# sharonct/CTPA-CLIP

Hardware: AMD Instinct MI355X
Metric: CT-report pairs/sec (contrastive step) (higher is better)
Workload: dtype bf16

## Files before the change

ctpa-clip_amd/csrc/gemm.hip:

```cpp
#include <algorithm>
#include "common.h"
#include "../../include/ctclip_hip.h"

int ctclip_gemm256(const ctclip_gemm_args* a, int split, int batch, void* stream);

namespace {

constexpr int BM = 128, BN = 128, BKT = 64, NTH = 256;
constexpr int KROW = BKT * 2 + 16;
constexpr int TILE_BYTES = 128 * KROW;
constexpr int SMEM_BYTES = 4 * TILE_BYTES;
constexpr int CS_LD = 132;

struct P {
  int64_t M, N, K;
  const u16* A; int64_t lda;
  const u16* B; int64_t ldb;
  const u16* B2;
  void* C; int64_t ldc; int c_f32;
  u16* C2; int64_t ldc2;
  const float* bias;
  const void* R; int64_t ldr; int r_f32;
  float alpha; int act; int accumulate; int split_k;
  int64_t sA, sB, sC, sC2, sR;
  int64_t kper;
  int r_f16;
};

__device__ __forceinline__ int mn_swz(int k) { return (k & 3) | (((k >> 3) & 1) << 2); }

template <bool KC>
__device__ __forceinline__ void gload(u32x4 (&r)[4], const u16* __restrict__ base, int64_t ld,
                                      int64_t rows, int64_t kend, int64_t row0, int64_t k0) {
  const int t = threadIdx.x;
  if constexpr (KC) {
    const int kc = t & 7;
    const int64_t gk = k0 + kc * 8;
#pragma unroll
    for (int i = 0; i < 4; ++i) {
      const int64_t gr = row0 + (t >> 3) + 32 * i;
      if (gr < rows && gk < kend) r[i] = *(const u32x4*)(base + gr * ld + gk);
      else r[i] = make_uint4(0, 0, 0, 0);
    }
  } else {
    const int mc = t & 15;
    const int64_t gm = row0 + mc * 8;
#pragma unroll
    for (int i = 0; i < 4; ++i) {
      const int64_t gk = k0 + (t >> 4) + 16 * i;
      if (gk < kend && gm < rows) r[i] = *(const u32x4*)(base + gk * ld + gm);
      else r[i] = make_uint4(0, 0, 0, 0);
    }
  }
}

template <bool KC>
__device__ __forceinline__ void swrite(char* tile, const u32x4 (&r)[4]) {
  const int t = threadIdx.x;
  if constexpr (KC) {
    const int kc = t & 7;
#pragma unroll
    for (int i = 0; i < 4; ++i) *(u32x4*)(tile + ((t >> 3) + 32 * i) * KROW + kc * 16) = r[i];
  } else {
    const int mc = t & 15, c32 = mc >> 1, half = mc & 1;
#pragma unroll
    for (int i = 0; i < 4; ++i) {
      const int kk = (t >> 4) + 16 * i;
      *(u32x4*)(tile + kk * 256 + ((((c32 ^ mn_swz(kk)) << 1) | half) << 4)) = r[i];
    }
  }
}
// ... 2 lines not shown
__device__ __forceinline__ bf16x8 frag(const char* tile, int r0, int s, int lane) {
  if constexpr (KC) {
    const int row = r0 + (lane & 15);
    return *(const bf16x8*)(tile + row * KROW + ((s * 4 + (lane >> 4)) << 4));
  } else {
    const int g = lane >> 4, i = lane & 15, q = i >> 2, p = i & 3;
    const int m = r0 + 4 * p;
    const int k1 = s * 32 + 8 * g + q, k2 = k1 + 4;
    const int c32 = m >> 4, within = (m & 15) * 2;
    const int o1 = k1 * 256 + ((c32 ^ mn_swz(k1)) << 5) + within;
    const int o2 = k2 * 256 + ((c32 ^ mn_swz(k2)) << 5) + within;
    s16x4 lo = __builtin_amdgcn_ds_read_tr16_b64_v4i16(LDS_PTR(s16x4, tile + o1));
    s16x4 hi = __builtin_amdgcn_ds_read_tr16_b64_v4i16(LDS_PTR(s16x4, tile + o2));
    typedef short s16x8 __attribute__((ext_vector_type(8)));
    s16x8 v = {lo[0], lo[1], lo[2], lo[3], hi[0], hi[1], hi[2], hi[3]};
    return __builtin_bit_cast(bf16x8, v);
  }
}

__device__ __forceinline__ void xcd_remap(int& tx, int& ty) {
  const int gx = gridDim.x, nwg = gridDim.x * gridDim.y;
  const int orig = blockIdx.y * gx + blockIdx.x;
  int id = orig;
  if (nwg >= 16) {
    const int xcd = orig & 7, q = nwg >> 3, r = nwg & 7;
    id = (xcd < r ? xcd * (q + 1) : r * (q + 1) + (xcd - r) * q) + (orig >> 3);
  }
  ty = id / gx;
  tx = id - ty * gx;
}

template <bool AK, bool BK, bool H16 = false>
__global__ __launch_bounds__(NTH, 2) void gemm_kernel(P p) {
  extern __shared__ __attribute__((aligned(16))) char smem[];
  const int lane = threadIdx.x & 63, w = threadIdx.x >> 6, wr = w >> 1, wc = w & 1;
  int tx, ty;
  xcd_remap(tx, ty);
  const int split = blockIdx.z % p.split_k, bidx = blockIdx.z / p.split_k;
  const int64_t m0 = (int64_t)ty * BM, n0 = (int64_t)tx * BN;
  const int64_t kbeg = split * p.kper;
  const int64_t kend = min(p.K, kbeg + p.kper);
  const u16* A = p.A + bidx * p.sA;
  const u16* B = p.B + bidx * p.sB;
#define AS(i) (smem + (i) * TILE_BYTES)
#define BS(i) (smem + (2 + (i)) * TILE_BYTES)

  f32x4 acc[4][4];
#pragma unroll
  for (int i = 0; i < 4; ++i)
#pragma unroll
    for (int j = 0; j < 4; ++j) acc[i][j] = f32x4{0.f, 0.f, 0.f, 0.f};

  u32x4 ra[4], rb[4];
  const int nk1 = kend > kbeg ? (int)((kend - kbeg + BKT - 1) / BKT) : 0;
  const int nk = p.B2 ? 2 * nk1 : nk1;
  const u16* B2 = p.B2 ? p.B2 + bidx * p.sB : nullptr;
  if (nk > 0) {
    gload<AK>(ra, A, p.lda, p.M, kend, m0, kbeg);
    gload<BK>(rb, B, p.ldb, p.N, kend, n0, kbeg);
    swrite<AK>(AS(0), ra);
    swrite<BK>(BS(0), rb);
  }
  __syncthreads();
  for (int kt = 0; kt < nk; ++kt) {
    const int cur = kt & 1;
    if (kt + 1 < nk) {
      const int kn = kt + 1 < nk1 ? kt + 1 : kt + 1 - nk1;
      gload<AK>(ra, A, p.lda, p.M, kend, m0, kbeg + (int64_t)kn * BKT);
      gload<BK>(rb, kt + 1 < nk1 ? B : B2, p.ldb, p.N, kend, n0, kbeg + (int64_t)kn * BKT);
    }
#pragma unroll
    for (int s = 0; s < 2; ++s) {
      bf16x8 af[4], bfr[4];
#pragma unroll
      for (int i = 0; i < 4; ++i) af[i] = frag<AK>(AS(cur), wr * 64 + i * 16, s, lane);
#pragma unroll
      for (int j = 0; j < 4; ++j) bfr[j] = frag<BK>(BS(cur), wc * 64 + j * 16, s, lane);
#pragma unroll
      for (int i = 0; i < 4; ++i)
#pragma unroll
        for (int j = 0; j < 4; ++j)
          acc[i][j] = mfma16<H16>(af[i], bfr[j], acc[i][j]);
    }
    if (kt + 1 < nk) {
      swrite<AK>(AS(cur ^ 1), ra);
      swrite<BK>(BS(cur ^ 1), rb);
    }
    __syncthreads();
  }

  float* cs = (float*)smem;
#pragma unroll
  for (int i = 0; i < 4; ++i)
#pragma unroll
    for (int j = 0; j < 4; ++j)
#pragma unroll
      for (int r = 0; r < 4; ++r)
        cs[(wr * 64 + i * 16 + (lane >> 4) * 4 + r) * CS_LD + wc * 64 + j * 16 + (lane & 15)] = acc[i][j][r];
  __syncthreads();

  const int t = threadIdx.x;
  if (p.act == 3) {
    const int row = t >> 1, half = t & 1;
    const int ncol = (int)min((int64_t)BN, p.N - n0);
    float best = -INFINITY, second = -INFINITY;
    int bi = 0x7fffffff;
    for (int c = half * 64; c < half * 64 + 64; ++c) {
      const float v = cs[row * CS_LD + c];
      if (c < ncol) {
        if (v > best) { second = best; best = v; bi = c; }
        else if (v > second) second = v;
      }
    }
    const int64_t gm = m0 + row;
    if (gm < p.M && half * 64 < ncol) {
      float2* out = (float2*)p.C + bidx * p.sC;
      out[gm * p.ldc + tx * 2 + half] = make_float2(best, __int_as_float((int)(n0 + bi)));
      if (p.C2) ((float*)p.C2)[bidx * p.sC2 + gm * p.ldc2 + tx * 2 + half] = second;
    }
    return;
  }
  const bool slab = p.split_k > 1;
// ... 243 lines not shown
    for (int j = 0; j < 4; ++j) { v[j] += a[j]; v[4 + j] += b[j]; }
  }
  if (drop) {
#pragma unroll
    for (int j = 0; j < 8; ++j) v[j] *= hid_keep(seed, r * cols + c + j, thresh, dscale);
  }
  if (p.R) {
    if (p.r_f32) {
      const float* Rp = (const float*)p.R + r * p.ldr + c;
      const f32x4 a = *(const f32x4*)Rp, b = *(const f32x4*)(Rp + 4);
#pragma unroll
      for (int j = 0; j < 4; ++j) { v[j] += a[j]; v[4 + j] += b[j]; }
    } else {
      float rr[8];
      unpack8(*(const u32x4*)((const u16*)p.R + r * p.ldr + c), rr);
#pragma unroll
      for (int j = 0; j < 8; ++j) v[j] += rr[j];
    }
  }
  if (p.act == 1) {
    if (p.C2) *(u32x4*)(p.C2 + r * p.ldc2 + c) = pack8(v);
#pragma unroll
    for (int j = 0; j < 8; ++j) v[j] = gelu_erf(v[j]);
  }
  if (p.c_f32) {
    float* Cf = (float*)p.C + r * p.ldc + c;
    if (p.accumulate) {
      const f32x4 a = *(const f32x4*)Cf, b = *(const f32x4*)(Cf + 4);
#pragma unroll
      for (int j = 0; j < 4; ++j) { v[j] += a[j]; v[4 + j] += b[j]; }
    }
    *(f32x4*)Cf = f32x4{v[0], v[1], v[2], v[3]};
    *(f32x4*)(Cf + 4) = f32x4{v[4], v[5], v[6], v[7]};
  } else {
    u16* Cb = (u16*)p.C + r * p.ldc + c;
    if (p.accumulate) {
      float rr[8];
      unpack8(*(const u32x4*)Cb, rr);
#pragma unroll
      for (int j = 0; j < 8; ++j) v[j] += rr[j];
    }
    *(u32x4*)Cb = pack8(v);
  }
  if (p.C2 && p.act == 0) *(u32x4*)(p.C2 + r * p.ldc2 + c) = pack8(v);
}

static bool s_smem_set = false;

}

extern "C" int ctclip_gemm(const ctclip_gemm_args* a, void* stream) {
  if (!a) return CT_EINVAL;
  if (a->M <= 0 || a->N <= 0 || a->K <= 0) return a->M == 0 || a->N == 0 ? 0 : CT_ESHAPE;
  const int split = a->split_k > 0 ? a->split_k : 1;
  if (split > 1 && !a->c_f32) return CT_EINVAL;
  if (a->act == 2 && !a->C2) return CT_EINVAL;
  CT_REQUIRE(aligned16(a->A) && aligned16(a->B) && aligned16(a->C), CT_EALIGN);
  CT_REQUIRE(a->lda % 8 == 0 && a->ldb % 8 == 0, CT_EALIGN);
  CT_REQUIRE(a->a_kcontig ? (a->K % 8 == 0) : (a->M % 8 == 0), CT_EALIGN);
  CT_REQUIRE(a->b_kcontig ? (a->K % 8 == 0) : (a->N % 8 == 0), CT_EALIGN);
  if (a->act != 3) {
    CT_REQUIRE(a->N % 8 == 0 && a->ldc % 8 == 0, CT_EALIGN);
    if (a->C2) CT_REQUIRE(aligned16(a->C2) && a->ldc2 % 8 == 0, CT_EALIGN);
    if (a->R) CT_REQUIRE(aligned16(a->R) && a->ldr % 8 == 0, CT_EALIGN);
  }
  if (a->act == 2) CT_REQUIRE(a->N % 64 == 0 && a->ldc2 % 8 == 0, CT_ESHAPE);
  if (a->act == 4) CT_REQUIRE(a->N % 32 == 0 && a->R && !a->r_f32 && !a->c_f32 && a->split_k <= 1, CT_EINVAL);
  if (a->act == 6)
    CT_REQUIRE(a->R && !a->r_f32 && !a->bias && !a->accumulate && !a->C2 && split == 1 && (a->batch <= 1), CT_EINVAL);
  if (a->act == 5)
    CT_REQUIRE(a->C2 && a->bias && aligned16(a->bias) && !a->R && !a->c_f32 && !a->accumulate && split == 1 &&
                   (a->batch <= 1) && a->N % 64 == 0 && a->n2 > 0 && a->n2 % 64 == 0 && a->n2 <= a->N,
               CT_EINVAL);
  if (a->B2) CT_REQUIRE(aligned16(a->B2) && a->act != 3, CT_EINVAL);
  if (a->A_lo || a->B_lo) {
    CT_REQUIRE(a->A_lo && a->B_lo && a->ab_f16 && aligned16(a->A_lo) && aligned16(a->B_lo) && a->K % 64 == 0,
               CT_EINVAL);
    CT_REQUIRE(a->a_kcontig && a->b_kcontig && !a->B2 && split == 1 && !a->accumulate && a->batch <= 1, CT_EINVAL);
    CT_REQUIRE(a->K < (int64_t)64 * 10000, CT_ESHAPE);
    if (a->act == 2)
      CT_REQUIRE(!a->c_f32 && !a->R && !a->bias && a->C3 && aligned16(a->C3) && a->ldc3 % 8 == 0 &&
                     (!a->C4 || (aligned16(a->C4) && a->ldc4 % 8 == 0)),
                 CT_EINVAL);
    else
      CT_REQUIRE(a->act == 0 && a->c_f32 && (!a->R || a->r_f32), CT_EINVAL);
    return ctclip_gemm256(a, 1, 1, stream);
  }
  if (a->ab_f16)
    CT_REQUIRE(a->a_kcontig && a->b_kcontig && !a->B2 && split == 1 && (a->act == 0 || a->act == 2 || a->act == 3) &&
                   !a->accumulate && (a->batch <= 1),
               CT_EINVAL);
  if (!a->B2 && a->act != 6) {
    const int b = a->batch > 0 ? a->batch : 1;
    const int64_t tiles256 = ((a->M + 255) / 256) * ((a->N + 255) / 256) * split * b;
    if (a->K % 64 == 0 && a->M >= 256 && a->N >= 256 && tiles256 >= 160 && (split == 1 || (a->K / split) >= 512) &&
        (!a->bias || aligned16(a->bias)))
      return ctclip_gemm256(a, split, b, stream);
  }
  if (a->act == 5) {
    ctclip_gemm_args g = *a;
    g.act = 0;
    g.bias = nullptr;
    g.C2 = nullptr;
    const int rc = ctclip_gemm(&g, stream);
    if (rc) return rc;
    return ctclip_l2norm_scale_fwd(a->C, a->ldc, a->M, a->n2 / 32, 32, a->bias, a->C2, a->ldc2, stream);
  }
  if (!s_smem_set) {
    (void)hipFuncSetAttribute((const void*)gemm_kernel<true, true>, hipFuncAttributeMaxDynamicSharedMemorySize, SMEM_BYTES);
    (void)hipFuncSetAttribute((const void*)gemm_kernel<true, false>, hipFuncAttributeMaxDynamicSharedMemorySize, SMEM_BYTES);
    (void)hipFuncSetAttribute((const void*)gemm_kernel<false, true>, hipFuncAttributeMaxDynamicSharedMemorySize, SMEM_BYTES);
    (void)hipFuncSetAttribute((const void*)gemm_kernel<false, false>, hipFuncAttributeMaxDynamicSharedMemorySize, SMEM_BYTES);
    (void)hipFuncSetAttribute((const void*)gemm_kernel<true, true, true>, hipFuncAttributeMaxDynamicSharedMemorySize, SMEM_BYTES);
    s_smem_set = true;
  }
  P p;
  p.M = a->M; p.N = a->N; p.K = a->K;
  p.A = (const u16*)a->A; p.lda = a->lda;
  p.B = (const u16*)a->B; p.ldb = a->ldb;
  p.B2 = (const u16*)a->B2;
  p.C = a->C; p.ldc = a->ldc; p.c_f32 = a->c_f32;
  p.C2 = (u16*)a->C2; p.ldc2 = a->ldc2;
  p.bias = a->bias;
  p.R = a->R; p.ldr = a->ldr; p.r_f32 = a->r_f32;
  p.alpha = a->alpha; p.act = a->act; p.accumulate = a->accumulate; p.split_k = split;
  p.sA = a->sA; p.sB = a->sB; p.sC = a->sC; p.sC2 = a->sC2; p.sR = a->sR;
  int64_t kper = (a->K + split - 1) / split;
  kper = (kper + BKT - 1) / BKT * BKT;
  p.kper = kper;
  p.r_f16 = a->r_f16;
  const int batch = a->batch > 0 ? a->batch : 1;
  hipStream_t st = (hipStream_t)stream;
  if (a->ab_f16) return launch<true, true, true>(p, batch, st);
  if (a->a_kcontig && a->b_kcontig) return launch<true, true>(p, batch, st);
  if (a->a_kcontig && !a->b_kcontig) return launch<true, false>(p, batch, st);
  if (!a->a_kcontig && a->b_kcontig) return launch<false, true>(p, batch, st);
  return launch<false, false>(p, batch, st);
}

extern "C" int ctclip_reduce_slabs_ep(const float* slabs, int64_t nslab, int64_t rows, int64_t cols, int64_t ld,
                                      const ctclip_gemm_args* a, void* stream) {
  if (rows == 0 || cols == 0) return 0;
  CT_REQUIRE(a && (a->act == 0 || a->act == 1), CT_EINVAL);
  CT_REQUIRE(cols % 8 == 0 && ld % 4 == 0 && a->ldc % 8 == 0 && aligned16(slabs) && aligned16(a->C), CT_EALIGN);
  if (a->bias) CT_REQUIRE(aligned16(a->bias), CT_EALIGN);
  if (a->R) CT_REQUIRE(aligned16(a->R) && a->ldr % 8 == 0, CT_EALIGN);
  if (a->C2) CT_REQUIRE(aligned16(a->C2) && a->ldc2 % 8 == 0, CT_EALIGN);
  P p{};
  p.C = a->C; p.ldc = a->ldc; p.c_f32 = a->c_f32;
  p.C2 = (u16*)a->C2; p.ldc2 = a->ldc2;
  p.bias = a->bias;
  p.R = a->R; p.ldr = a->ldr; p.r_f32 = a->r_f32;
  p.act = a->act; p.accumulate = a->accumulate;
  const int64_t total = rows * (cols / 8);
  hipLaunchKernelGGL(reduce_slabs_ep_kernel, dim3(cdiv(total, 256)), dim3(256), 0, (hipStream_t)stream, slabs, nslab,
                     rows, cols, ld, p);
  CT_CHECK_LAUNCH();
  return 0;
}

extern "C" int ctclip_reduce_slabs_ep_drop(const float* slabs, int64_t nslab, int64_t rows, int64_t cols, int64_t ld,
                                           const ctclip_gemm_args* a, float dp, uint64_t seed, void* stream) {
  if (rows == 0 || cols == 0) return 0;
  CT_REQUIRE(a && a->act == 0 && !a->accumulate && a->ldc == cols && dp >= 0.f && dp < 1.f, CT_EINVAL);
  CT_REQUIRE(cols % 8 == 0 && ld % 4 == 0 && aligned16(slabs) && aligned16(a->C), CT_EALIGN);
  if (a->bias) CT_REQUIRE(aligned16(a->bias), CT_EALIGN);
  if (a->R) CT_REQUIRE(aligned16(a->R) && a->ldr % 8 == 0, CT_EALIGN);
  if (a->C2) CT_REQUIRE(aligned16(a->C2) && a->ldc2 % 8 == 0, CT_EALIGN);
  P p{};
  p.C = a->C; p.ldc = a->ldc; p.c_f32 = a->c_f32;
  p.C2 = (u16*)a->C2; p.ldc2 = a->ldc2;
  p.bias = a->bias;
  p.R = a->R; p.ldr = a->ldr; p.r_f32 = a->r_f32;
// ... 92 lines not shown
```

ctpa-clip_amd/ctclip_mi355x/_lib.py:

```python
from __future__ import annotations

import ctypes
import os

import torch

_HERE = os.path.dirname(os.path.abspath(__file__))
LIB_PATH = os.environ.get('CTCLIP_HIP_LIB') or os.path.join(_HERE, 'libctclip_hip.so')
_LIB = None

c_i64 = ctypes.c_int64
c_i32 = ctypes.c_int32
c_f32 = ctypes.c_float
c_vp = ctypes.c_void_p


class SlabJob(ctypes.Structure):
    _fields_ = [('slabs', c_vp), ('nslab', c_i64), ('cols', c_i64), ('out', c_vp), ('accumulate', c_i32),
                ('pad', c_i32)]


ABI_VERSION = 2


# ... 102 lines not shown

class ClipLossExArgs(ctypes.Structure):
    _fields_ = [
        ('t_raw', c_vp), ('i_raw', c_vp), ('t_extra', c_vp), ('i_extra', c_vp), ('log_temp', c_vp),
        ('Vt', c_i32), ('Vi', c_i32), ('Bg', c_i32), ('Dl', c_i32),
        ('decoupled', c_i32), ('w_main', c_f32), ('w_multiview', c_f32),
        ('loss', c_vp), ('pair_loss', c_vp),
        ('dt_raw', c_vp), ('di_raw', c_vp), ('dt_extra', c_vp), ('di_extra', c_vp),
        ('dlogtemp', c_vp),
        ('ws', c_vp), ('ws_floats', c_i64),
    ]


class ClipLossTiledArgs(ctypes.Structure):
    _fields_ = ClipLossExArgs._fields_[:-1] + [('ws_bytes', c_i64), ('grad_row0', c_i32), ('grad_rows', c_i32)]


class MlmMaskArgs(ctypes.Structure):
    _fields_ = [
        ('ids', c_vp), ('B', c_i32), ('L', c_i32),
        ('num_tokens', c_i64), ('mask_token_id', c_i64), ('pad_token_id', c_i64),
        ('ignore', c_i64 * 32), ('n_ignore', c_i32), ('m_max', c_i32),
        ('mask_prob', ctypes.c_double), ('replace_prob', ctypes.c_double), ('random_token_prob', ctypes.c_double),
        ('seed', ctypes.c_uint64),
        ('masked_ids', c_vp), ('labels', c_vp), ('sel', c_vp),
    ]


_SIGS = {
    'ctclip_version': [],
    'ctclip_device_arch': [ctypes.c_char_p, c_i32],
    'ctclip_debug_hold_cus': [c_i32, c_i64, c_i32, c_vp],
    'ctclip_gemm': [ctypes.POINTER(GemmArgs), c_vp],
    'ctclip_gemm_ln': [ctypes.POINTER(GemmArgs), ctypes.POINTER(LnEpilogueArgs), c_vp],
    'ctclip_gemm_qkv_lnfold': [ctypes.POINTER(GemmArgs), c_vp, c_vp, c_vp, c_i32, c_vp],
    'ctclip_gemm_qkv_lnfold2': [ctypes.POINTER(GemmArgs), c_vp, c_vp, c_vp, c_i32, c_i32, c_vp],
    'ctclip_pack_qkv_fold': [c_vp, c_i64, c_vp, c_i64, c_i64, c_vp, c_i64, c_i64, c_vp, c_i64, c_vp, c_vp, c_vp,
                             c_i32, c_vp, c_vp],
    'ctclip_ln_stats_merge': [c_vp, c_i32, c_i64, c_i32, c_f32, c_vp, c_vp, c_vp],
    'ctclip_lnfold_wgrad': [c_vp, c_i64, c_vp, c_vp, c_vp, c_i64, c_i64, c_i64, c_i64, c_vp, c_i64, c_vp, c_vp,
                            c_i64, c_vp],
    'ctclip_gemm_lnfold_bwd': [ctypes.POINTER(GemmArgs), c_vp, c_i64, c_vp, c_vp, c_vp],
    'ctclip_l2norm_qk_bwd_fold': [c_vp, c_i64, c_vp, c_i64, c_i64, c_vp, c_vp, c_vp, c_i64, c_vp, c_i32, c_vp, c_vp,
                                  c_vp, c_vp, c_i32, c_vp, c_vp, c_vp],
    'ctclip_quant_mxfp8': [c_vp, c_i32, c_i64, c_i64, c_i64, c_vp, c_i64, c_vp, c_i64, c_vp],
    'ctclip_gemm_mxfp8': [ctypes.POINTER(MxGemmArgs), c_vp],
    'ctclip_gemm_mxfp8_set_tile': [c_i32],
    'ctclip_dropout': [c_vp, c_vp, c_vp, c_vp, c_i64, c_f32, ctypes.c_uint64, c_vp],
    'ctclip_gemm_set_variant': [c_i32],
    'ctclip_gemm_set_stagger': [c_i32],
    'ctclip_gemm_set_epi_lds': [c_i32],
    'ctclip_gemm_set_persist': [c_i32],
    'ctclip_gemm_set_grid_cap': [c_i32],
    'ctclip_reduce_slabs_ep': [c_vp, c_i64, c_i64, c_i64, c_i64, ctypes.POINTER(GemmArgs), c_vp],
    'ctclip_reduce_slabs_ep_drop': [c_vp, c_i64, c_i64, c_i64, c_i64, ctypes.POINTER(GemmArgs), c_f32, ctypes.c_uint64,
                                    c_vp],
    'ctclip_layernorm_bwd_drop': [c_vp, c_i32, c_i64, c_vp, c_i32, c_i64, c_vp, c_vp, c_vp, c_i64, c_i32, c_vp, c_i64,
                                  c_vp, c_i64, c_vp, c_vp, c_vp, c_i32, c_f32, ctypes.c_uint64, c_vp],
    'ctclip_patch_ln_x2': [c_vp, c_i32, c_i32, c_i64, c_i32, c_i32, c_i32, c_i32, c_i32, c_i32, c_vp, c_f32, c_vp,
                           c_vp, c_i64, c_vp],
    'ctclip_patch_ln_x3': [c_vp, c_i32, c_i32, c_i64, c_i32, c_i32, c_i32, c_i32, c_i32, c_i32, c_vp, c_f32, c_vp,
                           c_vp, c_vp, c_i64, c_vp],
    'ctclip_layernorm_fwd_x2': [c_vp, c_i32, c_i64, c_i64, c_i32, c_vp, c_vp, c_f32, c_vp, c_vp, c_i64, c_vp, c_i64,
                                c_vp, c_vp, c_vp],
    'ctclip_layernorm_fwd_x3': [c_vp, c_i32, c_i64, c_i64, c_i32, c_vp, c_vp, c_f32, c_vp, c_vp, c_vp, c_i64, c_vp,
                                c_i64, c_vp, c_vp, c_vp, c_vp],
    'ctclip_pack_rows_h16': [c_vp, c_i64, c_vp, c_i64, c_i32, c_i32, c_vp, c_vp, c_i64, c_vp],
    'ctclip_pack_qkv_fold_h16': [c_vp, c_i64, c_vp, c_i64, c_i64, c_vp, c_i64, c_i64, c_vp, c_i64, c_vp, c_vp],
    'ctclip_skinny_gemm_slices': [c_i64, c_i64, c_i64],
    'ctclip_skinny_gemm': [c_vp, c_i64, c_vp, c_i64, c_i64, c_i64, c_i64, c_vp, c_i32, c_vp],
    'ctclip_vq_l2norm_h16': [c_vp, c_i64, c_i64, c_i32, c_vp, c_i64, c_vp],
    'ctclip_skinny_sgemm_slices': [c_i64, c_i64, c_i64],
    'ctclip_skinny_sgemm': [c_vp, c_i64, c_vp, c_i64, c_i64, c_i64, c_i64, c_vp, c_i32, c_vp],
    'ctclip_reduce_slabs': [c_vp, c_i64, c_i64, c_i64, c_i64, c_vp, c_i64, c_i32, c_i32, c_vp],
    'ctclip_reduce_slabs_multi': [ctypes.POINTER(SlabJob), c_i32, c_vp],
    'ctclip_layernorm_fwd': [c_vp, c_i32, c_i64, c_i64, c_i32, c_vp, c_vp, c_f32, c_vp, c_i64, c_vp, c_i64,
                             c_vp, c_vp, c_vp],
    'ctclip_layernorm_bwd': [c_vp, c_i32, c_i64, c_vp, c_i32, c_i64, c_vp, c_vp, c_vp, c_i64, c_i32, c_vp, c_i64,
                             c_vp, c_i64, c_vp, c_i64, c_vp, c_vp, c_i32, c_vp],
    'ctclip_l2norm_scale_fwd': [c_vp, c_i64, c_i64, c_i32, c_i32, c_vp, c_vp, c_i64, c_vp],
    'ctclip_l2norm_scale_bwd': [c_vp, c_i64, c_vp, c_i64, c_i64, c_i32, c_i32, c_vp, c_vp, c_i64, c_vp, c_i32, c_vp],
    'ctclip_l2norm_scale_bwd_fold': [c_vp, c_i64, c_vp, c_i64, c_i64, c_i32, c_i32, c_vp, c_vp, c_i64, c_vp, c_i32,
                                     c_vp, c_vp, c_vp, c_i64, c_vp, c_vp, c_i32, c_vp, c_vp, c_vp],
    'ctclip_colsum': [c_vp, c_i32, c_i64, c_i64, c_i32, c_vp, c_i32, c_vp],
    'ctclip_geglu_bwd': [c_vp, c_i64, c_vp, c_i64, c_i64, c_i32, c_vp, c_i64, c_vp],
    'ctclip_gelu_bwd': [c_vp, c_vp, c_vp, c_i64, c_vp],
    'ctclip_pack_rows': [c_vp, c_i64, c_vp, c_i64, c_i32, c_i32, c_vp, c_vp, c_i64, c_vp],
    'ctclip_pack_rows_f32': [c_vp, c_i64, c_vp, c_i64, c_i32, c_i32, c_vp, c_vp, c_i64, c_vp],
    'ctclip_split_f16': [c_vp, c_i64, c_i64, c_i32, c_f32, c_vp, c_vp, c_i64, c_vp, c_vp],
    'ctclip_pack_rows_x3': [c_vp, c_i64, c_vp, c_i64, c_i32, c_i32, c_vp, c_f32, c_vp, c_vp, c_i64, c_vp, c_vp],
    'ctclip_sgemm_tn': [ctypes.POINTER(SgemmTnArgs), c_vp],
    'ctclip_unpack_rows': [c_vp, c_i64, c_vp, c_i64, c_i32, c_vp, c_i64, c_i32, c_vp],
    'ctclip_reduce_slabs_rows': [c_vp, c_i64, c_i64, c_i64, c_i64, c_vp, c_vp, c_i64, c_i32, c_vp],
    'ctclip_gelu_f32': [c_vp, c_vp, c_i64, c_vp],
    'ctclip_cast_f32_bf16': [c_vp, c_vp, c_i64, c_vp],
    'ctclip_cast_f32_bf16_split': [c_vp, c_vp, c_vp, c_i64, c_vp],
    'ctclip_add_f32': [c_vp, c_vp, c_vp, c_vp, c_i64, c_vp],
    'ctclip_patch_ln': [c_vp, c_i32, c_i32, c_i64, c_i32, c_i32, c_i32, c_i32, c_i32, c_i32, c_vp, c_f32, c_vp, c_i64,
                        c_vp],
    'ctclip_patch_wgrad': [c_vp, c_vp, c_vp, c_vp, c_vp, c_i32, c_i32, c_vp, c_vp, c_vp, c_i32, c_vp],
    'ctclip_unpatch_mse': [c_vp, c_i64, c_vp, c_i32, c_i32, c_i64, c_i32, c_i32, c_i32, c_i32, c_i32, c_i32, c_vp,
                           c_vp, c_i64, c_vp, c_vp, c_vp, c_vp],
    'ctclip_peg_fwd': [c_vp, c_vp, c_i64, c_i32, c_i32, c_i32, c_i32, c_vp, c_vp, c_i32, c_vp, c_vp, c_vp],
    'ctclip_peg_fwd_stats': [c_vp, c_vp, c_i64, c_i32, c_i32, c_i32, c_i32, c_vp, c_vp, c_i32, c_vp, c_vp, c_vp,
                             c_vp],
    'ctclip_peg_fwd_x32': [c_vp, c_i64, c_i32, c_i32, c_i32, c_i32, c_vp, c_vp, c_i32, c_vp, c_vp, c_vp, c_vp, c_vp],
# ... 115 lines not shown
```

ctpa-clip_amd/ctclip_mi355x/kernels.py:

```python
from __future__ import annotations

import os

import torch

from . import _lib
from ._lib import GemmArgs, LnEpilogueArgs, call, ptr, stream_ptr

BF16 = torch.bfloat16
F32 = torch.float32
F16 = torch.float16

ACT_NONE, ACT_GELU, ACT_GEGLU, ACT_ARGMAX, ACT_GEGLU_BWD, ACT_L2N, ACT_GELU_BWD = 0, 1, 2, 3, 4, 5, 6


def _chk(t, name, dtype=None):
    if not t.is_cuda:
        raise ValueError(f'{name}: expected a device tensor')
    if dtype is not None and t.dtype != dtype:
        raise ValueError(f'{name}: expected {dtype}, got {t.dtype}')


class KernelTimer:

    def __init__(self):
        self.active = False
        self.tags = set()
        self.events = []

    def start(self, tags):
        self.active, self.tags, self.events = True, set(tags), []

    def stop(self):
        self.active = False

    def __call__(self, tag, flops):
        if not (self.active and tag in self.tags):
            return None
        s, e = torch.cuda.Event(enable_timing=True), torch.cuda.Event(enable_timing=True)
        s.record()
        self.events.append((tag, s, e, flops))
        return e

    def summary(self, tag):
        torch.cuda.synchronize()
        ev = [(s, e, f) for t, s, e, f in self.events if t == tag]
        if not ev:
            return None
        ms = [s.elapsed_time(e) for s, e, _ in ev]
        return dict(launches=len(ev), avg_ms=sum(ms) / len(ms), flops=ev[0][2], total_ms=sum(ms),
                    total_flops=sum(f for _, _, f in ev))


TIMER = KernelTimer()


def gemm_raw(M, N, K, A, lda, a_kcontig, B, ldb, b_kcontig, C, ldc, *, C2=None, ldc2=0, bias=None,
             R=None, ldr=0, alpha=1.0, act=ACT_NONE, accumulate=False, split_k=1, batch=1,
             sA=0, sB=0, sC=0, sC2=0, sR=0, tag=None, flops=None, n2=0, B2=None, drop=None):
    end = TIMER(tag, flops if flops is not None else 2.0 * M * N * K * batch) if tag else None
    _gemm_raw(M, N, K, A, lda, a_kcontig, B, ldb, b_kcontig, C, ldc, C2=C2, ldc2=ldc2, bias=bias, R=R, ldr=ldr,
              alpha=alpha, act=act, accumulate=accumulate, split_k=split_k, batch=batch, sA=sA, sB=sB, sC=sC,
              sC2=sC2, sR=sR, n2=n2, B2=B2, drop=drop)
    if end is not None:
        end.record()


def _gemm_raw(M, N, K, A, lda, a_kcontig, B, ldb, b_kcontig, C, ldc, *, C2=None, ldc2=0, bias=None,
              R=None, ldr=0, alpha=1.0, act=ACT_NONE, accumulate=False, split_k=1, batch=1,
              sA=0, sB=0, sC=0, sC2=0, sR=0, n2=0, B2=None, drop=None):
    if B2 is not None:
        assert B2.dtype == B.dtype and B2.shape == B.shape and B2.stride() == B.stride()
    h16 = A.dtype == F16
    assert B.dtype == A.dtype, (A.dtype, B.dtype)
    s = 1 if h16 else _auto_split(M, N, K, act, split_k, batch, accumulate, C)
    if drop is not None:
        assert act == ACT_NONE and not accumulate and C.dtype == F32 and batch == 1 and ldc == N
        if s <= 1:
            _gemm_raw(M, N, K, A, lda, a_kcontig, B, ldb, b_kcontig, C, ldc, bias=bias, alpha=alpha, B2=B2)
            call('ctclip_dropout', ptr(C), ptr(R), ptr(C), ptr(C2), M * N, float(drop[0]),
                 int(drop[1]) & (2 ** 64 - 1), stream_ptr())
            return
        slabs = torch.empty(s, M, N, device=C.device, dtype=F32)
        _gemm_raw(M, N, K, A, lda, a_kcontig, B, ldb, b_kcontig, slabs, N, alpha=alpha, split_k=s, B2=B2)
        a = GemmArgs()
        a.C, a.ldc, a.c_f32 = ptr(C), ldc, 1
        a.C2, a.ldc2 = ptr(C2), ldc2
        a.bias = ptr(bias)
        a.R, a.ldr, a.r_f32 = ptr(R), ldr, int(R is not None and R.dtype == F32)
        call('ctclip_reduce_slabs_ep_drop', ptr(slabs), s, M, N, N, _lib.ctypes.byref(a), float(drop[0]),
             int(drop[1]) & (2 ** 64 - 1), stream_ptr())
        return
    if s > 1:
        slabs = torch.empty(s, M, N, device=C.device, dtype=F32)
        _gemm_raw(M, N, K, A, lda, a_kcontig, B, ldb, b_kcontig, slabs, N, alpha=alpha, split_k=s, B2=B2)
        a = GemmArgs()
        a.C, a.ldc, a.c_f32 = ptr(C), ldc, int(C.dtype == F32)
        a.C2, a.ldc2 = ptr(C2), ldc2
        a.bias = ptr(bias)
        a.R, a.ldr, a.r_f32 = ptr(R), ldr, int(R is not None and R.dtype == F32)
        a.act, a.accumulate = act, int(accumulate)
        call('ctclip_reduce_slabs_ep', ptr(slabs), s, M, N, N, _lib.ctypes.byref(a), stream_ptr())
        return
    a = GemmArgs()
    a.M, a.N, a.K = M, N, K
    a.A, a.lda, a.a_kcontig = ptr(A), lda, int(a_kcontig)
    a.B, a.ldb, a.b_kcontig = ptr(B), ldb, int(b_kcontig)
    a.C, a.ldc, a.c_f32 = ptr(C), ldc, int(C.dtype == F32)
    a.C2, a.ldc2 = ptr(C2), ldc2
    a.bias = ptr(bias)
    a.R, a.ldr, a.r_f32 = ptr(R), ldr, int(R is not None and R.dtype == F32)
    a.alpha, a.act, a.accumulate, a.split_k, a.batch = alpha, act, int(accumulate), split_k, batch
    a.sA, a.sB, a.sC, a.sC2, a.sR = sA, sB, sC, sC2, sR
    a.n2 = n2
    a.B2 = ptr(B2)
    a.ab_f16 = int(h16)
    a.r_f16 = int(R is not None and R.dtype == F16)
    call('ctclip_gemm', _lib.ctypes.byref(a), stream_ptr())


def _auto_split(M, N, K, act, split_k, batch, accumulate, C):
    if split_k != 1 or batch != 1 or act not in (ACT_NONE, ACT_GELU) or K < 512 or N % 8 or C.stride(-1) != 1:
        return 1
    tiles = ((M + 127) // 128) * ((N + 127) // 128)
    if tiles >= 128 or M * N > (1 << 22):
        return 1
    return max(1, min(256 // tiles, K // 256))


def linear(x, w, *, bias=None, residual=None, out=None, out_dtype=BF16, act=ACT_NONE, out2=None, alpha=1.0,
           accumulate=False, tag=None, flops=None, l2n_scale=None, l2n_cols=0, w_lo=None, dropout=None,
           discard_out=False):
    M, K = x.shape
    N = w.shape[0]
    assert w.shape[1] == K and x.stride(1) == 1 and w.stride(1) == 1
    if discard_out:
        assert act == ACT_GEGLU and x.dtype == F16 and out2 is not None and out is None
        a = GemmArgs()
        a.M, a.N, a.K = M, N, K
        a.A, a.lda, a.a_kcontig = ptr(x), x.stride(0), 1
        a.B, a.ldb, a.b_kcontig = ptr(w), w.stride(0), 1
        a.C, a.ldc = None, N
        a.C2, a.ldc2 = ptr(out2), out2.stride(0)
        a.alpha, a.act, a.split_k, a.batch, a.ab_f16 = alpha, ACT_GEGLU, 1, 1, 1
        end = TIMER(tag, flops if flops is not None else 2.0 * M * N * K) if tag else None
        call('ctclip_gemm', _lib.ctypes.byref(a), stream_ptr())
        if end is not None:
            end.record()
        return None
    if out is None:
        out = torch.empty(M, N, device=x.device, dtype=out_dtype)
    if l2n_scale is not None:
        assert bias is None and residual is None and out2 is not None and l2n_scale.numel() == 32
        assert l2n_scale.dtype == torch.float32 and l2n_scale.is_contiguous()
        act, bias = ACT_L2N, l2n_scale
    gemm_raw(M, N, K, x, x.stride(0), True, w, w.stride(0), True, out, out.stride(0),
             C2=out2, ldc2=out2.stride(0) if out2 is not None else 0, bias=bias, R=residual,
             ldr=residual.stride(0) if residual is not None else 0, alpha=alpha, act=act, accumulate=accumulate,
             tag=tag, flops=flops, n2=l2n_cols, B2=w_lo, drop=dropout)
    return out


def matmul_nn(dy, w, *, out=None, out_dtype=BF16, residual=None, accumulate=False, alpha=1.0):
    M, N = dy.shape
    K = w.shape[1]
    assert w.shape[0] == N
    if out is None:
        out = torch.empty(M, K, device=dy.device, dtype=out_dtype)
# ... 1432 lines not shown
```

include/ctclip_hip.h:

```cpp
#ifndef CTCLIP_HIP_H
#define CTCLIP_HIP_H
#include <stdint.h>
#ifdef __cplusplus
extern "C" {
#endif

#define CTCLIP_ABI_VERSION 2
#define CT_STATUS_LN_TIMEOUT 1
#define CT_STATUS_F16_RANGE 2
#define CT_STATUS_NONFINITE_GRAD 4
#define CT_STATUS_VQ_NONFINITE 8
int ctclip_version(void);
int ctclip_device_arch(char* buf, int n);
int ctclip_debug_hold_cus(int32_t nwg, int64_t cycles, int32_t lds_bytes, void* stream);

typedef struct {
  int64_t M, N, K;
  const void* A; int64_t lda; int32_t a_kcontig;
  const void* B; int64_t ldb; int32_t b_kcontig;
  void* C; int64_t ldc; int32_t c_f32;
  void* C2; int64_t ldc2;
  const float* bias;
  const void* R; int64_t ldr; int32_t r_f32;
  float alpha;
  int32_t act;
  int32_t accumulate;
  int32_t split_k;
  int32_t batch;
  int64_t sA, sB, sC, sC2, sR;
  int32_t n2;
  const void* B2;
  int32_t ab_f16;
  int32_t r_f16;
  const void* A_lo;
  const void* B_lo;
  void* C3; int64_t ldc3;
  void* C4; int64_t ldc4;
} ctclip_gemm_args;
int ctclip_gemm(const ctclip_gemm_args* a, void* stream);
int ctclip_gemm_set_variant(int variant);
int ctclip_gemm_set_stagger(int units);
int ctclip_gemm_set_epi_lds(int on);
int ctclip_gemm_set_persist(int on);
int ctclip_gemm_set_grid_cap(int workgroups);

int ctclip_reduce_slabs_ep_drop(const float* slabs, int64_t nslab, int64_t rows, int64_t cols, int64_t ld,
                                const ctclip_gemm_args* ep, float p, uint64_t seed, void* stream);
int ctclip_layernorm_bwd_drop(const void* dy, int32_t dy_f32, int64_t lddy, const void* x, int32_t x_f32, int64_t ldx,
                              const float* mean, const float* rstd, const float* gamma, int64_t rows, int32_t D,
                              float* dx_f32, int64_t lddxf, void* dx_bf16, int64_t lddxb, float* part_gamma,
                              float* part_beta, float* part_drop, int32_t nblocks, float p, uint64_t seed,
                              void* stream);

typedef struct {
  int32_t mode;
  const float* gamma; const float* beta; float eps;
  void* Y; int64_t ldy;
  float* mean; float* rstd;
  const void* X; int64_t ldx;
  float* part_gamma; float* part_beta;
  void* xchg; uint32_t epoch;
  int32_t* status;
  uint32_t spin_limit;
  int32_t debug;
  void* Y16;
} ctclip_ln_epilogue;
int ctclip_gemm_ln(const ctclip_gemm_args* a, const ctclip_ln_epilogue* ln, void* stream);

int ctclip_gemm_qkv_lnfold(const ctclip_gemm_args* a, const float* mean, const float* rstd, const float* fold_cs,
                           int32_t nfold, void* stream);
int ctclip_gemm_qkv_lnfold2(const ctclip_gemm_args* a, const float* mean, const float* rstd, const float* fold_cs,
                            int32_t nfold, int32_t c_col0, void* stream);
int ctclip_pack_qkv_fold(const float* Wq, int64_t ldq, const float* gamma, int64_t nq, int64_t K,
                         const void* Wrest, int64_t ldr, int64_t nrest, void* out, int64_t ldo, float* cs,
                         const float* s_fold, const float* s_rest, int32_t ns, float* s_out, void* stream);
int ctclip_pack_qkv_fold_h16(const float* Wq, int64_t ldq, const float* gamma, int64_t nq, int64_t K,
                             const float* Wrest, int64_t ldr, int64_t nrest, void* out, int64_t ldo, float* cs,
                             void* stream);
int ctclip_ln_stats_merge(const float* part, int32_t ngroups, int64_t rows, int32_t D, float eps, float* mean,
                          float* rstd, void* stream);
int ctclip_gemm_lnfold_bwd(const ctclip_gemm_args* a, const void* X, int64_t ldx, const float* c1, const float* beta,
                           void* stream);
int ctclip_lnfold_wgrad(const float* G, int64_t ldg, const float* u, const float* gamma, const float* Wq, int64_t ldw,
                        int64_t nq, int64_t nrest, int64_t K, float* grad_q, int64_t ldgq, float* grad_gamma,
                        float* grad_rest, int64_t ldgr, void* stream);

int ctclip_skinny_gemm_slices(int64_t M, int64_t N, int64_t K);
int ctclip_skinny_gemm(const void* A, int64_t lda, const void* B, int64_t ldb, int64_t M, int64_t N, int64_t K,
                       float* slabs, int32_t nslices, void* stream);
int ctclip_skinny_sgemm_slices(int64_t M, int64_t N, int64_t K);
int ctclip_skinny_sgemm(const float* A, int64_t lda, const float* B, int64_t ldb, int64_t M, int64_t N, int64_t K,
                        float* slabs, int32_t nslices, void* stream);
// ... 332 lines not shown
```

Before: 211.5.

## Add dedicated hi/lo split-weight GEMM kernel with fused dropout epilogue

Hi/lo split-B GEMMs, where A is multiplied by B and by a low-order residual B2, move out of the generic 128x128 kernel, which walked K twice over B then B2. A new 64x64 kernel loads A once per K tile, keeps both B and B2 tiles in LDS, and issues MFMAs for both into the same accumulators. It uses a three-stage register ring and an epilogue that can apply dropout in place. This removes the second pass over A, the separate dropout kernel and the split-K slab path for these calls. The trade-off is smaller tiles, which mean less reuse per tile, and the hi/lo case no longer uses split-K.

```diff
diff --git a/ctpa-clip_amd/csrc/gemm.hip b/ctpa-clip_amd/csrc/gemm.hip
--- a/ctpa-clip_amd/csrc/gemm.hip
+++ b/ctpa-clip_amd/csrc/gemm.hip
@@ -16,7 +16,6 @@
   int64_t M, N, K;
   const u16* A; int64_t lda;
   const u16* B; int64_t ldb;
-  const u16* B2;
   void* C; int64_t ldc; int c_f32;
   u16* C2; int64_t ldc2;
   const float* bias;
@@ -125,9 +124,7 @@
     for (int j = 0; j < 4; ++j) acc[i][j] = f32x4{0.f, 0.f, 0.f, 0.f};
 
   u32x4 ra[4], rb[4];
-  const int nk1 = kend > kbeg ? (int)((kend - kbeg + BKT - 1) / BKT) : 0;
-  const int nk = p.B2 ? 2 * nk1 : nk1;
-  const u16* B2 = p.B2 ? p.B2 + bidx * p.sB : nullptr;
+  const int nk = kend > kbeg ? (int)((kend - kbeg + BKT - 1) / BKT) : 0;
   if (nk > 0) {
     gload<AK>(ra, A, p.lda, p.M, kend, m0, kbeg);
     gload<BK>(rb, B, p.ldb, p.N, kend, n0, kbeg);
@@ -138,9 +135,8 @@
   for (int kt = 0; kt < nk; ++kt) {
     const int cur = kt & 1;
     if (kt + 1 < nk) {
-      const int kn = kt + 1 < nk1 ? kt + 1 : kt + 1 - nk1;
-      gload<AK>(ra, A, p.lda, p.M, kend, m0, kbeg + (int64_t)kn * BKT);
-      gload<BK>(rb, kt + 1 < nk1 ? B : B2, p.ldb, p.N, kend, n0, kbeg + (int64_t)kn * BKT);
+      gload<AK>(ra, A, p.lda, p.M, kend, m0, kbeg + (int64_t)(kt + 1) * BKT);
+      gload<BK>(rb, B, p.ldb, p.N, kend, n0, kbeg + (int64_t)(kt + 1) * BKT);
     }
 #pragma unroll
     for (int s = 0; s < 2; ++s) {
@@ -490,6 +486,7 @@
 extern "C" int ctclip_gemm(const ctclip_gemm_args* a, void* stream) {
   if (!a) return CT_EINVAL;
   if (a->M <= 0 || a->N <= 0 || a->K <= 0) return a->M == 0 || a->N == 0 ? 0 : CT_ESHAPE;
+  if (a->B2) return ctclip_gemm_hilo(a, 0.f, 0, stream);
   const int split = a->split_k > 0 ? a->split_k : 1;
   if (split > 1 && !a->c_f32) return CT_EINVAL;
   if (a->act == 2 && !a->C2) return CT_EINVAL;
@@ -510,11 +507,10 @@
     CT_REQUIRE(a->C2 && a->bias && aligned16(a->bias) && !a->R && !a->c_f32 && !a->accumulate && split == 1 &&
                    (a->batch <= 1) && a->N % 64 == 0 && a->n2 > 0 && a->n2 % 64 == 0 && a->n2 <= a->N,
                CT_EINVAL);
-  if (a->B2) CT_REQUIRE(aligned16(a->B2) && a->act != 3, CT_EINVAL);
   if (a->A_lo || a->B_lo) {
     CT_REQUIRE(a->A_lo && a->B_lo && a->ab_f16 && aligned16(a->A_lo) && aligned16(a->B_lo) && a->K % 64 == 0,
                CT_EINVAL);
-    CT_REQUIRE(a->a_kcontig && a->b_kcontig && !a->B2 && split == 1 && !a->accumulate && a->batch <= 1, CT_EINVAL);
+    CT_REQUIRE(a->a_kcontig && a->b_kcontig && split == 1 && !a->accumulate && a->batch <= 1, CT_EINVAL);
     CT_REQUIRE(a->K < (int64_t)64 * 10000, CT_ESHAPE);
     if (a->act == 2)
       CT_REQUIRE(!a->c_f32 && !a->R && !a->bias && a->C3 && aligned16(a->C3) && a->ldc3 % 8 == 0 &&
@@ -525,10 +521,10 @@
     return ctclip_gemm256(a, 1, 1, stream);
   }
   if (a->ab_f16)
-    CT_REQUIRE(a->a_kcontig && a->b_kcontig && !a->B2 && split == 1 && (a->act == 0 || a->act == 2 || a->act == 3) &&
+    CT_REQUIRE(a->a_kcontig && a->b_kcontig && split == 1 && (a->act == 0 || a->act == 2 || a->act == 3) &&
                    !a->accumulate && (a->batch <= 1),
                CT_EINVAL);
-  if (!a->B2 && a->act != 6) {
+  if (a->act != 6) {
     const int b = a->batch > 0 ? a->batch : 1;
     const int64_t tiles256 = ((a->M + 255) / 256) * ((a->N + 255) / 256) * split * b;
     if (a->K % 64 == 0 && a->M >= 256 && a->N >= 256 && tiles256 >= 160 && (split == 1 || (a->K / split) >= 512) &&
@@ -556,7 +552,6 @@
   p.M = a->M; p.N = a->N; p.K = a->K;
   p.A = (const u16*)a->A; p.lda = a->lda;
   p.B = (const u16*)a->B; p.ldb = a->ldb;
-  p.B2 = (const u16*)a->B2;
   p.C = a->C; p.ldc = a->ldc; p.c_f32 = a->c_f32;
   p.C2 = (u16*)a->C2; p.ldc2 = a->ldc2;
   p.bias = a->bias;
diff --git a/ctpa-clip_amd/csrc/gemm_hilo.hip b/ctpa-clip_amd/csrc/gemm_hilo.hip
--- /dev/null
+++ b/ctpa-clip_amd/csrc/gemm_hilo.hip
@@ -0,0 +1,242 @@
+#include <algorithm>
+#include "common.h"
+#include "../../include/ctclip_hip.h"
+
+namespace {
+
+constexpr int BM = 64, BN = 64, BKT = 64, NTH = 256;
+constexpr int KROW = BKT * 2 + 16;
+constexpr int TILE_BYTES = BM * KROW;
+constexpr int SMEM_BYTES = 3 * TILE_BYTES;
+constexpr int CS_LD = BN + 4;
+constexpr int RING = 3;
+static_assert(BM * CS_LD * 4 <= SMEM_BYTES, "epilogue staging reuses the operand tiles");
+
+struct HP {
+  int64_t M, N, K;
+  const u16* A; int64_t lda;
+  const u16* Bh; const u16* Bl; int64_t ldb;
+  void* C; int64_t ldc; int c_f32;
+  u16* C2; int64_t ldc2;
+  const float* bias;
+  const void* R; int64_t ldr; int r_f32;
+  float alpha; int act; int accumulate;
+  unsigned thresh; float dscale; uint64_t seed; int drop;
+};
+
+struct Stage {
+  u32x4 a[2], h[2], l[2];
+};
+
+__device__ __forceinline__ bool in_tile(int64_t rows, int64_t kend, int64_t row0, int64_t k0, int i) {
+  const int t = threadIdx.x;
+  return row0 + (t >> 3) + 32 * i < rows && k0 + (t & 7) * 8 < kend;
+}
+
+__device__ __forceinline__ void gload(u32x4 (&r)[2], const u16* __restrict__ base, int64_t ld, int64_t rows,
+                                      int64_t kend, int64_t row0, int64_t k0) {
+  const int t = threadIdx.x;
+#pragma unroll
+  for (int i = 0; i < 2; ++i) {
+    const u16* src = base + (row0 + (t >> 3) + 32 * i) * ld + k0 + (t & 7) * 8;
+    r[i] = *(const u32x4*)(in_tile(rows, kend, row0, k0, i) ? src : base);
+  }
+}
+
+__device__ __forceinline__ void swrite(char* tile, const u32x4 (&r)[2], int64_t rows, int64_t kend, int64_t row0,
+                                       int64_t k0) {
+  const int t = threadIdx.x;
+#pragma unroll
+  for (int i = 0; i < 2; ++i)
+    *(u32x4*)(tile + ((t >> 3) + 32 * i) * KROW + (t & 7) * 16) =
+        in_tile(rows, kend, row0, k0, i) ? r[i] : make_uint4(0, 0, 0, 0);
+}
+
+__device__ __forceinline__ bf16x8 frag(const char* tile, int r0, int s, int lane) {
+  return *(const bf16x8*)(tile + (r0 + (lane & 15)) * KROW + ((s * 4 + (lane >> 4)) << 4));
+}
+
+__device__ __forceinline__ void xcd_remap(int& tx, int& ty) {
+  const int gx = gridDim.x, nwg = gridDim.x * gridDim.y;
+  const int orig = blockIdx.y * gx + blockIdx.x;
+  int id = orig;
+  if (nwg >= 16) {
+    const int xcd = orig & 7, q = nwg >> 3, r = nwg & 7;
+    id = (xcd < r ? xcd * (q + 1) : r * (q + 1) + (xcd - r) * q) + (orig >> 3);
+  }
+  ty = id / gx;
+  tx = id - ty * gx;
+}
+
+__global__ __launch_bounds__(NTH) void gemm_hilo_kernel(HP p) {
+  __shared__ __attribute__((aligned(16))) char smem[SMEM_BYTES];
+  const int lane = threadIdx.x & 63, w = threadIdx.x >> 6, wr = w >> 1, wc = w & 1;
+  int tx, ty;
+  xcd_remap(tx, ty);
+  const int64_t m0 = (int64_t)ty * BM, n0 = (int64_t)tx * BN;
+  char* As = smem;
+  char* Hs = smem + TILE_BYTES;
+  char* Ls = smem + 2 * TILE_BYTES;
+
+  f32x4 acc[2][2];
+#pragma unroll
+  for (int i = 0; i < 2; ++i)
+#pragma unroll
+    for (int j = 0; j < 2; ++j) acc[i][j] = f32x4{0.f, 0.f, 0.f, 0.f};
+
+  const int nk = (int)((p.K + BKT - 1) / BKT);
+  Stage st[RING];
+  auto load = [&](Stage& s, int kt) {
+    const int64_t k0 = (int64_t)kt * BKT;
+    gload(s.a, p.A, p.lda, p.M, p.K, m0, k0);
+    gload(s.h, p.Bh, p.ldb, p.N, p.K, n0, k0);
+    gload(s.l, p.Bl, p.ldb, p.N, p.K, n0, k0);
+  };
+  auto write = [&](const Stage& s, int kt) {
+    const int64_t k0 = (int64_t)kt * BKT;
+    swrite(As, s.a, p.M, p.K, m0, k0);
+    swrite(Hs, s.h, p.N, p.K, n0, k0);
+    swrite(Ls, s.l, p.N, p.K, n0, k0);
+  };
+#pragma unroll
+  for (int u = 0; u < RING; ++u) load(st[u], u);
+  write(st[0], 0);
+  __syncthreads();
+  for (int kb = 0; kb < nk; kb += RING) {
+#pragma unroll
+    for (int u = 0; u < RING; ++u) {
+      const int kt = kb + u;
+      if (kt >= nk) break;
+      load(st[u], kt + RING);
+#pragma unroll
+      for (int s = 0; s < 2; ++s) {
+        bf16x8 af[2], bh[2], bl[2];
+#pragma unroll
+        for (int i = 0; i < 2; ++i) af[i] = frag(As, wr * 32 + i * 16, s, lane);
+#pragma unroll
+        for (int j = 0; j < 2; ++j) {
+          bh[j] = frag(Hs, wc * 32 + j * 16, s, lane);
+          bl[j] = frag(Ls, wc * 32 + j * 16, s, lane);
+        }
+#pragma unroll
+        for (int i = 0; i < 2; ++i)
+#pragma unroll
+          for (int j = 0; j < 2; ++j) acc[i][j] = __builtin_amdgcn_mfma_f32_16x16x32_bf16(af[i], bh[j], acc[i][j], 0, 0, 0);
+#pragma unroll
+        for (int i = 0; i < 2; ++i)
+#pragma unroll
+          for (int j = 0; j < 2; ++j) acc[i][j] = __builtin_amdgcn_mfma_f32_16x16x32_bf16(af[i], bl[j], acc[i][j], 0, 0, 0);
+      }
+      __syncthreads();
+      if (kt + 1 < nk) write(st[(u + 1) % RING], kt + 1);
+      __syncthreads();
+    }
+  }
+
+  float* cs = (float*)smem;
+#pragma unroll
+  for (int i = 0; i < 2; ++i)
+#pragma unroll
+    for (int j = 0; j < 2; ++j)
+#pragma unroll
+      for (int r = 0; r < 4; ++r)
+        cs[(wr * 32 + i * 16 + (lane >> 4) * 4 + r) * CS_LD + wc * 32 + j * 16 + (lane & 15)] = acc[i][j][r];
+  __syncthreads();
+
+  const int t = threadIdx.x;
+#pragma unroll
+  for (int it = 0; it < (BM * BN / 8) / NTH; ++it) {
+    const int c = t + NTH * it;
+    const int row = c >> 3, cc = (c & 7) * 8;
+    const int64_t gm = m0 + row, gn = n0 + cc;
+    if (gm >= p.M || gn >= p.N) continue;
+    float v[8];
+    const f32x4 lo = *(const f32x4*)(cs + row * CS_LD + cc);
+    const f32x4 hi = *(const f32x4*)(cs + row * CS_LD + cc + 4);
+#pragma unroll
+    for (int j = 0; j < 4; ++j) { v[j] = lo[j] * p.alpha; v[4 + j] = hi[j] * p.alpha; }
+    if (p.bias) {
+      const f32x4 a = *(const f32x4*)(p.bias + gn), b = *(const f32x4*)(p.bias + gn + 4);
+#pragma unroll
+      for (int j = 0; j < 4; ++j) { v[j] += a[j]; v[4 + j] += b[j]; }
+    }
+    if (p.drop) {
+#pragma unroll
+      for (int j = 0; j < 8; ++j) v[j] *= hid_keep(p.seed, gm * p.N + gn + j, p.thresh, p.dscale);
+    }
+    if (p.R) {
+      if (p.r_f32) {
+        const float* Rp = (const float*)p.R + gm * p.ldr + gn;
+        const f32x4 a = *(const f32x4*)Rp, b = *(const f32x4*)(Rp + 4);
+#pragma unroll
+        for (int j = 0; j < 4; ++j) { v[j] += a[j]; v[4 + j] += b[j]; }
+      } else {
+        float rr[8];
+        unpack8(*(const u32x4*)((const u16*)p.R + gm * p.ldr + gn), rr);
+#pragma unroll
+        for (int j = 0; j < 8; ++j) v[j] += rr[j];
+      }
+    }
+    if (p.act == 1) {
+      if (p.C2) *(u32x4*)(p.C2 + gm * p.ldc2 + gn) = pack8(v);
+#pragma unroll
+      for (int j = 0; j < 8; ++j) v[j] = gelu_erf(v[j]);
+    }
+    if (p.c_f32) {
+      float* Cf = (float*)p.C + gm * p.ldc + gn;
+      if (p.accumulate) {
+        const f32x4 a = *(const f32x4*)Cf, b = *(const f32x4*)(Cf + 4);
+#pragma unroll
+        for (int j = 0; j < 4; ++j) { v[j] += a[j]; v[4 + j] += b[j]; }
+      }
+      *(f32x4*)Cf = f32x4{v[0], v[1], v[2], v[3]};
+      *(f32x4*)(Cf + 4) = f32x4{v[4], v[5], v[6], v[7]};
+    } else {
+      u16* Cb = (u16*)p.C + gm * p.ldc + gn;
+      if (p.accumulate) {
+        float rr[8];
+        unpack8(*(const u32x4*)Cb, rr);
+#pragma unroll
+        for (int j = 0; j < 8; ++j) v[j] += rr[j];
+      }
+      *(u32x4*)Cb = pack8(v);
+    }
+    if (p.C2 && p.act == 0) *(u32x4*)(p.C2 + gm * p.ldc2 + gn) = pack8(v);
+  }
+}
+
+}
+
+extern "C" int ctclip_gemm_hilo(const ctclip_gemm_args* a, float dp, uint64_t seed, void* stream) {
+  if (!a) return CT_EINVAL;
+  if (a->M <= 0 || a->N <= 0 || a->K <= 0) return a->M == 0 || a->N == 0 ? 0 : CT_ESHAPE;
+  CT_REQUIRE(a->B2 && a->a_kcontig && a->b_kcontig && !a->ab_f16 && !a->A_lo && !a->B_lo, CT_EINVAL);
+  CT_REQUIRE((a->act == 0 || a->act == 1) && a->split_k <= 1 && a->batch <= 1, CT_EINVAL);
+  CT_REQUIRE(a->M < ((int64_t)1 << 31) - BM && a->N < ((int64_t)1 << 31) - BN && a->K < ((int64_t)1 << 31) - BKT,
+             CT_ESHAPE);
+  CT_REQUIRE(cdiv(a->M, BM) <= 65535, CT_ESHAPE);
+  CT_REQUIRE(aligned16(a->A) && aligned16(a->B) && aligned16(a->B2) && aligned16(a->C), CT_EALIGN);
+  CT_REQUIRE(a->lda % 8 == 0 && a->ldb % 8 == 0 && a->K % 8 == 0 && a->N % 8 == 0 && a->ldc % 8 == 0, CT_EALIGN);
+  if (a->bias) CT_REQUIRE(aligned16(a->bias), CT_EALIGN);
+  if (a->C2) CT_REQUIRE(aligned16(a->C2) && a->ldc2 % 8 == 0, CT_EALIGN);
+  if (a->R) CT_REQUIRE(aligned16(a->R) && a->ldr % 8 == 0, CT_EALIGN);
+  CT_REQUIRE(dp >= 0.f && dp < 1.f, CT_EINVAL);
+  if (dp > 0.f) CT_REQUIRE(a->act == 0 && !a->accumulate && a->ldc == a->N, CT_EINVAL);
+  HP p;
+  p.M = a->M; p.N = a->N; p.K = a->K;
+  p.A = (const u16*)a->A; p.lda = a->lda;
+  p.Bh = (const u16*)a->B; p.Bl = (const u16*)a->B2; p.ldb = a->ldb;
+  p.C = a->C; p.ldc = a->ldc; p.c_f32 = a->c_f32;
+  p.C2 = (u16*)a->C2; p.ldc2 = a->ldc2;
+  p.bias = a->bias;
+  p.R = a->R; p.ldr = a->ldr; p.r_f32 = a->r_f32;
+  p.alpha = a->alpha; p.act = a->act; p.accumulate = a->accumulate;
+  p.drop = dp > 0.f;
+  p.thresh = (unsigned)std::min(4294967295.0, (double)dp * 4294967296.0);
+  p.dscale = 1.f / (1.f - dp);
+  p.seed = seed;
+  dim3 grid(cdiv(a->N, BN), cdiv(a->M, BM));
+  hipLaunchKernelGGL(gemm_hilo_kernel, grid, dim3(NTH), 0, (hipStream_t)stream, p);
+  CT_CHECK_LAUNCH();
+  return 0;
+}
diff --git a/ctpa-clip_amd/ctclip_mi355x/_lib.py b/ctpa-clip_amd/ctclip_mi355x/_lib.py
--- a/ctpa-clip_amd/ctclip_mi355x/_lib.py
+++ b/ctpa-clip_amd/ctclip_mi355x/_lib.py
@@ -178,6 +178,7 @@
     'ctclip_gemm_set_epi_lds': [c_i32],
     'ctclip_gemm_set_persist': [c_i32],
     'ctclip_gemm_set_grid_cap': [c_i32],
+    'ctclip_gemm_hilo': [ctypes.POINTER(GemmArgs), c_f32, ctypes.c_uint64, c_vp],
     'ctclip_reduce_slabs_ep': [c_vp, c_i64, c_i64, c_i64, c_i64, ctypes.POINTER(GemmArgs), c_vp],
     'ctclip_reduce_slabs_ep_drop': [c_vp, c_i64, c_i64, c_i64, c_i64, ctypes.POINTER(GemmArgs), c_f32, ctypes.c_uint64,
                                     c_vp],
diff --git a/ctpa-clip_amd/ctclip_mi355x/kernels.py b/ctpa-clip_amd/ctclip_mi355x/kernels.py
--- a/ctpa-clip_amd/ctclip_mi355x/kernels.py
+++ b/ctpa-clip_amd/ctclip_mi355x/kernels.py
@@ -73,16 +73,31 @@
         assert B2.dtype == B.dtype and B2.shape == B.shape and B2.stride() == B.stride()
     h16 = A.dtype == F16
     assert B.dtype == A.dtype, (A.dtype, B.dtype)
+    if drop is not None:
+        assert act == ACT_NONE and not accumulate and C.dtype == F32 and batch == 1 and ldc == N
+    if B2 is not None:
+        assert a_kcontig and b_kcontig and not h16 and split_k == 1 and batch == 1
+        a = GemmArgs()
+        a.M, a.N, a.K = M, N, K
+        a.A, a.lda, a.a_kcontig = ptr(A), lda, 1
+        a.B, a.ldb, a.b_kcontig, a.B2 = ptr(B), ldb, 1, ptr(B2)
+        a.C, a.ldc, a.c_f32 = ptr(C), ldc, int(C.dtype == F32)
+        a.C2, a.ldc2 = ptr(C2), ldc2
+        a.bias = ptr(bias)
+        a.R, a.ldr, a.r_f32 = ptr(R), ldr, int(R is not None and R.dtype == F32)
+        a.alpha, a.act, a.accumulate, a.split_k, a.batch = alpha, act, int(accumulate), 1, 1
+        dp, seed = (float(drop[0]), int(drop[1]) & (2 ** 64 - 1)) if drop is not None else (0.0, 0)
+        call('ctclip_gemm_hilo', _lib.ctypes.byref(a), dp, seed, stream_ptr())
+        return
     s = 1 if h16 else _auto_split(M, N, K, act, split_k, batch, accumulate, C)
     if drop is not None:
-        assert act == ACT_NONE and not accumulate and C.dtype == F32 and batch == 1 and ldc == N
         if s <= 1:
-            _gemm_raw(M, N, K, A, lda, a_kcontig, B, ldb, b_kcontig, C, ldc, bias=bias, alpha=alpha, B2=B2)
+            _gemm_raw(M, N, K, A, lda, a_kcontig, B, ldb, b_kcontig, C, ldc, bias=bias, alpha=alpha)
             call('ctclip_dropout', ptr(C), ptr(R), ptr(C), ptr(C2), M * N, float(drop[0]),
                  int(drop[1]) & (2 ** 64 - 1), stream_ptr())
             return
         slabs = torch.empty(s, M, N, device=C.device, dtype=F32)
-        _gemm_raw(M, N, K, A, lda, a_kcontig, B, ldb, b_kcontig, slabs, N, alpha=alpha, split_k=s, B2=B2)
+        _gemm_raw(M, N, K, A, lda, a_kcontig, B, ldb, b_kcontig, slabs, N, alpha=alpha, split_k=s)
         a = GemmArgs()
         a.C, a.ldc, a.c_f32 = ptr(C), ldc, 1
         a.C2, a.ldc2 = ptr(C2), ldc2
@@ -93,7 +108,7 @@
         return
     if s > 1:
         slabs = torch.empty(s, M, N, device=C.device, dtype=F32)
-        _gemm_raw(M, N, K, A, lda, a_kcontig, B, ldb, b_kcontig, slabs, N, alpha=alpha, split_k=s, B2=B2)
+        _gemm_raw(M, N, K, A, lda, a_kcontig, B, ldb, b_kcontig, slabs, N, alpha=alpha, split_k=s)
         a = GemmArgs()
         a.C, a.ldc, a.c_f32 = ptr(C), ldc, int(C.dtype == F32)
         a.C2, a.ldc2 = ptr(C2), ldc2
@@ -113,7 +128,6 @@
     a.alpha, a.act, a.accumulate, a.split_k, a.batch = alpha, act, int(accumulate), split_k, batch
     a.sA, a.sB, a.sC, a.sC2, a.sR = sA, sB, sC, sC2, sR
     a.n2 = n2
-    a.B2 = ptr(B2)
     a.ab_f16 = int(h16)
     a.r_f16 = int(R is not None and R.dtype == F16)
     call('ctclip_gemm', _lib.ctypes.byref(a), stream_ptr())
diff --git a/include/ctclip_hip.h b/include/ctclip_hip.h
--- a/include/ctclip_hip.h
+++ b/include/ctclip_hip.h
@@ -38,6 +38,7 @@
   void* C4; int64_t ldc4;
 } ctclip_gemm_args;
 int ctclip_gemm(const ctclip_gemm_args* a, void* stream);
+int ctclip_gemm_hilo(const ctclip_gemm_args* a, float p, uint64_t seed, void* stream);
 int ctclip_gemm_set_variant(int variant);
 int ctclip_gemm_set_stagger(int units);
 int ctclip_gemm_set_epi_lds(int on);
```

New measurement: 211.1. Within noise of the previous version (-0.2%).
